# yenanjing/mmEgo

Hardware: AMD Instinct MI355X
Metric: train frames/sec (Upper+Lower U+L step, B=64/GPU, T=8, 128 pts) (higher is better)
Workload: dtype f32; 1 GPU; U+L step (Train_Upper + Train_Lower train_once bodies), B=64/GPU T=8 N=128, fp32, dropout live, two concurrent HIP-graph branches; global_batch=64, seq_len=8, points=128, parallelism=dp1

## Files before the change

### include/mmego_hip.h

```cpp
#ifndef MMEGO_HIP_H
#define MMEGO_HIP_H
#ifdef __cplusplus
extern "C" {
#endif

int mmego_gemm(void* stream, const float* A, long sam, long sak, const float* B, long sbk, long sbn, float* C,
               long scm, long scn, const float* bias, int M, int N, int K, int nbatch, long sAb, long sBb, long sCb,
               int relu, int accumulate, float* splitk_ws, int nsplit, long sBiasb, const float* cmul, float* asum);
typedef struct MmegoGemmDesc {
  const float* A; long sam, sak;
  const float* B; long sbk, sbn;
  float* C; long scm, scn;
  const float* bias;
  int M, N, K, nbatch;
  long sAb, sBb, sCb;
  int relu, accumulate;
  float* splitk_ws; int nsplit;
  long sBiasb;
  const float* cmul; float* asum;
} MmegoGemmDesc;
int mmego_gemm_group(void* stream, int n, const MmegoGemmDesc* descs);

int mmego_colstats_nblk(long rows);
int mmego_bn_train_stats(void* stream, const float* X, long ldx, long rows, int C, const float* gamma,
// ... 2 lines not shown
int mmego_bn_finalize(void* stream, const float* partial, int nblk, int C, const float* gamma, const float* beta,
                      float* running_mean, float* running_var, float momentum, float eps, float* mean, float* invstd, float* a,
                      float* b);
int mmego_bn_train_stats_pair(void* stream, long rows, int C, float* partial_ws,
                              const float* X1, long ldx1, const float* gamma1, const float* beta1, float* running_mean1,
                              float* running_var1, float momentum1, float eps1, float* mean1, float* invstd1, float* a1, float* b1,
                              const float* X2, long ldx2, const float* gamma2, const float* beta2, float* running_mean2,
                              float* running_var2, float momentum2, float eps2, float* mean2, float* invstd2, float* a2, float* b2);
int mmego_bn_eval_affine(void* stream, int C, const float* gamma, const float* beta, const float* running_mean,
                         const float* running_var, float eps, float* mean, float* invstd, float* a, float* b);
int mmego_bn_fold_linear(void* stream, const float* W, const float* b, int N, int K, const float* gamma, const float* beta,
                         const float* running_mean, const float* running_var, float eps, float* Wf, float* bf);
int mmego_mlp3_eval(void* stream, const float* X, long ldx, long rows, int Cin, const float* W1, const float* b1, int C1,
                    const float* W2, const float* b2, int C2, const float* W3, const float* b3, int C3, float* Y, long ldy,
                    const float* const* bn, float eps, int pre);
int mmego_mlp3_eval_bf16(void* stream, const float* X, long ldx, long rows, int Cin, const float* W1, const float* b1, int C1,
                         const float* W2, const float* b2, int C2, const float* W3, const float* b3, int C3, float* Y, long ldy,
                         const float* const* bn, float eps, int pre);
int mmego_affine_act(void* stream, const float* X1, long ld1, const float* m1, const float* a1, const float* b1,
                     const float* X2, long ld2, const float* m2, const float* a2, const float* b2, float* Y, long ldy,
                     long rows, int C, int relu);
int mmego_copy2d(void* stream, const float* X, long ldx, float* Y, long ldy, long rows, int C, int accumulate);
int mmego_gather_rows(void* stream, const float* X, long nsrc, long W, const long long* idx, long nout, float* Y);
int mmego_pack_frames(void* stream, const float* pts, const long long* frame_off, const long long* frame_idx, long nout,
                      int pc_no, int max_n, float keep_p, unsigned long long seed, float* out);
int mmego_pack_frames_noise(void* stream, const float* pts, const long long* frame_off, const long long* frame_idx, long nout,
                            int pc_no, int max_n, float keep_p, unsigned long long seed, float sigma_xyz, float sigma_v, float* out);
int mmego_pose_jitter(void* stream, const float* R, const float* t, long n, double sigma_deg, double sigma_t,
                      const long long* seed_word, const long long* ids, float* R_out, float* t_out);
int mmego_imu_jitter(void* stream, const float* imu, long n_rows, int T, int S,
                     double noise_rot_deg, double noise_acc, double noise_gyro,
                     double bias_rot_deg, double bias_acc, double bias_gyro,
                     const long long* seed_word, const long long* row_ids, const long long* win_ids,
                     float* out);
int mmego_blend_windows(void* stream, const float* src, long nrows, int C, const long long* cov_off, const int* cov_row,
                        const float* cov_w, long F, float* dst, long ldd, float* spread);
int mmego_colsum_phase(void* stream, const float* X, long ldx, long rows, int C, int period, float* out, long ldo);
int mmego_blend_bones(void* stream, const float* src, long nrows, int J, const long long* cov_off, const int* cov_row,
                      const float* cov_w, long F, const int* bones, const float* bone_len, int NB, float* dst, long ldd,
                      float* spread, int* fallback);
int mmego_bone_length_dev(void* stream, const float* X, long ldx, long n, int J, const int* bones, const float* bone_len, int NB,
                          float* out, long ldo);
int mmego_blend_rot(void* stream, const float* src, long nrows, int J, const float* q, int NQ, const float* Rh,
                    const long long* cov_off, const int* cov_row, const float* cov_w, long F, const int* bones, const int* rot_idx,
                    const float* body, int NB, float* dst, long ldd, float* quat, float* spread, float* rot_spread, int* fallback);
int mmego_smooth_frames(void* stream, const float* src, long lds, long F, int C, const int* seg, const float* w, int H, int D,
                        float* dst, long ldd, float* moved);
int mmego_smooth_bones(void* stream, const float* src, long lds, long F, int J, const int* seg, const float* w, int H, int D,
                       const int* bones, const float* bone_len, int NB, float* dst, long ldd, float* moved, int* fallback);
int mmego_floor_stats(void* stream, const float* lo, long ldl, const float* tgt, long ldt, const float* ground, const float* contact,
                      const int* seg, long rows, double H, float* out);
int mmego_floor_clamp(void* stream, const float* src, long lds, const float* ground, const int* seg, long rows, double margin, float* dst,
                      long ldd, float* lifted, int* fallback);
int mmego_bn_backward(void* stream, const float* dY, long lddy, const float* Ymask, long ldm, const float* X, long ldx,
                      const float* mean, const float* invstd, const float* a, long rows, int C, float* partial_ws,
                      float* c12_ws, float* dgamma, float* dbeta, float* dX, long lddx);
int mmego_bn_backward_pair(void* stream, const float* dY, long lddy, const float* Ymask, long ldm, long rows, int C,
                           float* partial_ws, float* c12_ws,
                           const float* X1, long ldx1, const float* mean1, const float* invstd1, const float* a1,
                           float* dgamma1, float* dbeta1, float* dX1, long lddx1,
                           const float* X2, long ldx2, const float* mean2, const float* invstd2, const float* a2,
                           float* dgamma2, float* dbeta2, float* dX2, long lddx2);
int mmego_colsum(void* stream, const float* X, long ldx, long rows, int C, float* partial_ws, float* out, float* out2,
                 int accumulate, const float* scale);
int mmego_colsum_pair(void* stream, const float* X, long ldx, long rows, int C, float* outA, float* outA2, float* outB,
                      float* outB2, int accumulate);
int mmego_relu_mask(void* stream, float* G, long ldg, const float* H, long ldh, long rows, int C);
int mmego_fill(void* stream, float* X, long n, float v);

int mmego_lstm_step(void* stream, int ndir, int Bn, int H, int first, const float* hprev0, const float* hprev1,
                    long hps, const float* whh0, const float* whh1, const float* bhh0, const float* bhh1,
                    const float* xproj0, const float* xproj1, long xs, float* hout0, float* hout1, long hos, float* c0,
                    float* c1, float* gst0, float* gst1, float* cst0, float* cst1);
int mmego_lstm64_forward(void* stream, int B, int T, const float* xproj0, const float* xproj1, long xs,
                         const float* whh0, const float* whh1, const float* bhh0, const float* bhh1, const float* h0_0,
                         const float* h0_1, const float* c0_0, const float* c0_1, float* out, long os, float* hn0,
                         float* hn1, float* cn0, float* cn1,
                         float* gates0, float* gates1, float* cst0, float* cst1, float* hprev0, float* hprev1,
                         float* drop_y, float* drop_mask, float drop_p, const unsigned long long* seed_ctr, int salt);
int mmego_lstm64_backward(void* stream, int B, int T, const float* dout, long dos, const float* gates0,
                          const float* gates1, const float* cst0, const float* cst1, const float* c0_0,
                          const float* c0_1, const float* whh0, const float* whh1, float* dgates0, float* dgates1,
                          long dgs);

typedef struct MmegoLstm64Fwd {
  const float* xproj[2]; long xs;
  const float* whh[2]; const float* bhh[2]; const float* h0[2]; const float* c0[2];
  float* out; long os;
  float* hn[2]; float* cn[2];
  float* gates[2]; float* cst[2]; float* hprev[2];
  int B, T;
  float* drop_y; float* drop_mask; float drop_p; const unsigned long long* seed_ctr; unsigned salt;
} MmegoLstm64Fwd;
typedef struct MmegoLstm64Bwd {
  const float* dout; long dos;
  const float* gates[2]; const float* cst[2]; const float* c0[2]; const float* whh[2];
  float* dgates[2]; long dgs;
  int B, T;
} MmegoLstm64Bwd;
int mmego_lstm64_forward_multi(void* stream, int n, const MmegoLstm64Fwd* descs);
int mmego_lstm64_backward_multi(void* stream, int n, const MmegoLstm64Bwd* descs);

int mmego_cvt_bf16(void* stream, const float* X, long ldx, long rows, long cols, unsigned short* Y, long ldy);
int mmego_cvt_bf16_tm(void* stream, const float* X, long ldx, int Bn, int T, long cols, unsigned short* Y, int Bp);
int mmego_gemm_bf16(void* stream, const unsigned short* A, long lda, const unsigned short* W, long ldw, float* C,
                    long ldc, unsigned short* Cb, long ldcb, float* Cf, const float* bias, int M, int N, int K, int relu);
int mmego_lstm_step_bf16(void* stream, int ndir, int Bn, int H, int first, const unsigned short* hprev0,
                         const unsigned short* hprev1, const unsigned short* whh0, const unsigned short* whh1,
                         const float* xpf, long mt0_0, long mt0_1, float* hout0, float* hout1,
                         long hos, unsigned short* houtb0, unsigned short* houtb1, long hbs,
                         unsigned short* hfrag0, unsigned short* hfrag1, float* c0, float* c1);

int mmego_lstm_step_bf16_fused(void* stream, int ndir, int Bn, int H, int first, int nseg,
                               const unsigned short* a0_0, const unsigned short* a0_1, const unsigned short* w0_0,
                               const unsigned short* w0_1, int K0, const unsigned short* a1_0,
                               const unsigned short* a1_1, const unsigned short* w1_0, const unsigned short* w1_1,
                               int K1, const unsigned short* hprev0, const unsigned short* hprev1,
                               const unsigned short* whh0, const unsigned short* whh1, const float* bias,
                               float* hout0, float* hout1, long hos, unsigned short* hfrag0, unsigned short* hfrag1,
                               float* c0, float* c1);
int mmego_attn_pool_frag_bf16_ok(int H);
int mmego_attn_pool_frag_bf16(void* stream, const unsigned short* hf, int T, int Bp, int Bn, int H, const float* w, const float* b,
                              float* vec, float* attn);
int mmego_cvt_bf16_frag_tm(void* stream, const float* X, long ldx, int Bn, int T, int C, unsigned short* Y, int Bp);
int mmego_fc_relu_bf16_frag_tm(void* stream, const float* X, long ldx, const float* W, const float* bias, int Bn, int T, int Cin,
                               int H, unsigned short* Y, int Bp, int relu);

int mmego_lstm_cell_backward(void* stream, int ndir, int Bn, int H, const float* dout0, const float* dout1, long dos,
                             const float* dhrec0, const float* dhrec1, const float* gst0, const float* gst1,
                             const float* cst0, const float* cst1, const float* cprev0, const float* cprev1, float* dc0,
                             float* dc1, float* dgates0, float* dgates1, long dgs);
int mmego_imu_loss(void* stream, const float* R, const float* t, const float* R_gt, const float* head_gt, long F,
                   float scale, float* loss, float* dR, float* dt);
int mmego_lstm_bwd_step(void* stream, int Bn, int H, const float* dg0, const float* dg1, long dgs, const float* wT0,
                        const float* wT1, const float* dout0, const float* dout1, long dos, const float* gst0,
                        const float* gst1, const float* cst0, const float* cst1, const float* cprev0, const float* cprev1,
                        float* dc0, float* dc1, float* dgo0, float* dgo1);
int mmego_imu_head_backward(void* stream, const float* y, const float* dR, const float* dt, long F, float* dy);

int mmego_transform2h(void* stream, float* pts, long F, int P, int C, const float* R, const float* t, const float* src,
                      long src_ld, float* keep, float* feats, long ldf, int nfeat);
int mmego_rotate_points(void* stream, const float* in, float* out, long F, int P, const float* R, const float* t,
                        int transpose, int add_t);
int mmego_transform2h_backward(void* stream, const float* pts, long ldp, long F, int P, const float* R, const float* t,
                               const float* g, long ldg, const float* g2, long ldg2, int accumulate, float* dR, float* dt);
int mmego_lower_inputs_backward(void* stream, const float* pts, long ldp, long F, int N, const long long* idx, int P, const float* R,
                                const float* t, const float* g, long ldg, const float* g2, long ldg2, const float* joints, int V,
                                const float* gj, long ldgj, const float* gj2, long ldgj2, int accumulate, float* dR, float* dt,
                                float* djoints);
int mmego_head_fk_forward(void* stream, int which, const float* y, const float* body, int B, long F, float* q,
                          float* joints, const float* Rw, const float* tw, float* world, long long* counters, int ncount,
                          unsigned long long* seed_ctr);
int mmego_head_fk_backward(void* stream, int which, const float* y, const float* body, int B, long F, const float* dj,
                           float* dy, const float* Rw);
int mmego_head_fk_backward_pose(void* stream, int which, const float* y, const float* body, int B, long F, const float* dj,
                                float* dy, const float* Rw, const float* joints_h, float* dRw, float* dtw);
int mmego_head_fk_backward_extra(void* stream, int which, const float* y, const float* body, int B, long F, const float* dj,
                                 float* dy, const float* Rw, const float* joints_h, float* dRw, float* dtw, const float* dR_add,
                                 const float* dt_add);
int mmego_head_fk_loss(void* stream, int which, const float* y, const float* body, int B, long F, float* q, float* joints_h,
                       const float* Rw, const float* tw, float* world, long long* counters, int ncount,
                       unsigned long long* seed_ctr, const float* target, const int* map, int ntgt, double scale, float* loss,
                       float* dy, double* scratch);
int mmego_head_fk_loss_pose(void* stream, int which, const float* y, const float* body, int B, long F, float* q, float* joints_h,
                            const float* Rw, const float* tw, float* world, long long* counters, int ncount,
                            unsigned long long* seed_ctr, const float* target, const int* map, int ntgt, double scale, float* loss,
// ... 257 lines not shown
```

### mmego_amd/csrc/lstm.hip

```cpp
#include "common.h"
#include "lstm_cell.h"
#include <stddef.h>
#include <string.h>

struct Lstm64P {
  const float* xproj[2]; long xs;
  const float* whh[2];
  const float* bhh[2];
  const float* h0[2]; const float* c0[2];
  float* out; long os;
  float* hn[2]; float* cn[2];
  float* gates[2]; float* cst[2]; float* hprev[2];
  int B, T;
  float* drop_y; float* drop_mask; float drop_p; const unsigned long long* seed_ctr; unsigned salt;
};
#define L64_SAME_FIELD(P, D, f) && offsetof(P, f) == offsetof(D, f) && sizeof(P::f) == sizeof(D::f)
#define L64_SAME_LAYOUT(P, D, FIELDS) static_assert(sizeof(P) == sizeof(D) FIELDS(L64_SAME_FIELD, P, D), #D " is " #P)
#define L64_FWD_FIELDS(X, P, D)                                                                                                        \
  X(P, D, xproj) X(P, D, xs) X(P, D, whh) X(P, D, bhh) X(P, D, h0) X(P, D, c0) X(P, D, out) X(P, D, os) X(P, D, hn) X(P, D, cn)       \
  X(P, D, gates) X(P, D, cst) X(P, D, hprev) X(P, D, B) X(P, D, T) X(P, D, drop_y) X(P, D, drop_mask) X(P, D, drop_p) X(P, D, seed_ctr) \
  X(P, D, salt)
L64_SAME_LAYOUT(Lstm64P, MmegoLstm64Fwd, L64_FWD_FIELDS);
template <class P, class D>
static inline P l64_param(const D& d) { P p; memcpy(&p, &d, sizeof p); return p; }


#define L64_LDS_BARRIER() asm volatile("s_waitcnt lgkmcnt(0)\n\ts_barrier" ::: "memory")

#define WLD 272

typedef const float __attribute__((address_space(1)))* l64_gcptr;
typedef float __attribute__((address_space(1)))* l64_gptr;
typedef f32x4 __attribute__((address_space(1)))* l64_gptr4;
typedef const f32x4 __attribute__((address_space(1)))* l64_gcptr4;

template <bool FULL, bool STASH, bool DROP>
__device__ __forceinline__ void lstm64_fwd_body(const Lstm64P& p) {
  extern __shared__ __attribute__((aligned(16))) float smem[];
  float* hs = smem;
  const int tid = threadIdx.x, lane = tid & 63, wave = tid >> 6;
  const int d = blockIdx.y, r0 = blockIdx.x * 16;
  const int B = p.B, T = p.T;
  const float* W = p.whh[d];
  const int fr = lane & 15, fq = lane >> 4;
  const int j = wave * 16 + fr;
  float creg[4], hreg[4], bh[4];
#pragma unroll
  for (int g = 0; g < 4; ++g) bh[g] = p.bhh[d] ? p.bhh[d][g * 64 + j] : 0.f;
#pragma unroll
  for (int reg = 0; reg < 4; ++reg) {
    int row = r0 + fq * 4 + reg;
    bool ok = row < B;
    creg[reg] = (ok && p.c0[d]) ? p.c0[d][row * 64 + j] : 0.f;
    hreg[reg] = (ok && p.h0[d]) ? p.h0[d][row * 64 + j] : 0.f;
    hs[j * 16 + fq * 4 + reg] = hreg[reg];
  }
  __syncthreads();
  float wreg[16][4];
#pragma unroll
  for (int g = 0; g < 4; ++g) {
    const float* wrow = W + (g * 64 + j) * 64 + 16 * fq;
#pragma unroll
    for (int q = 0; q < 4; ++q) {
      const f32x4 v = *reinterpret_cast<const f32x4*>(wrow + 4 * q);
      wreg[4 * q + 0][g] = v.x; wreg[4 * q + 1][g] = v.y; wreg[4 * q + 2][g] = v.z; wreg[4 * q + 3][g] = v.w;
    }
  }

  float xp[4][4], xpn[4][4];
  constexpr bool stash = STASH, keep_h = STASH, drop = DROP;
  const unsigned dkey = drop ? dropout_key(p.seed_ctr[0], p.salt) : 0u;
  const float keep_scale = drop ? 1.0f / (1.0f - p.drop_p) : 1.0f;
  const int t_first = d == 0 ? 0 : T - 1;
  const long dir = d == 0 ? 1 : -1;
  l64_gcptr xq[4];
  l64_gptr oq[4], hq[4], gq[4], cq[4];
  bool live[4];
#pragma unroll
  for (int reg = 0; reg < 4; ++reg) {
    const int row = r0 + fq * 4 + reg;
    live[reg] = FULL || row < B;
    const long rt = (long)(live[reg] ? row : 0) * T + t_first;
    xq[reg] = (l64_gcptr)(p.xproj[d] + rt * p.xs + j);
    oq[reg] = (l64_gptr)(p.out + rt * p.os + d * 64 + j);
    hq[reg] = keep_h ? (l64_gptr)(p.hprev[d] + rt * 64 + j) : (l64_gptr)nullptr;
    const long tr = (long)t_first * B + (live[reg] ? row : 0);
    gq[reg] = stash ? (l64_gptr)(p.gates[d] + tr * 256 + 4 * j) : (l64_gptr)nullptr;
    cq[reg] = stash ? (l64_gptr)(p.cst[d] + tr * 64 + j) : (l64_gptr)nullptr;
  }
  const long xstep = dir * p.xs, ostep = dir * p.os, hstep = dir * 64, gstep = dir * (long)B * 256,
             cstep = dir * (long)B * 64;
#define L64_LOAD_XP(DST)                                                                            \
  do {                                                                                              \
    _Pragma("unroll") for (int reg = 0; reg < 4; ++reg) {                                           \
      _Pragma("unroll") for (int g = 0; g < 4; ++g) DST[g][reg] = (FULL || live[reg]) ? xq[reg][g * 64] : 0.f; \
      xq[reg] += xstep;                                                                             \
    }                                                                                               \
  } while (0)
  L64_LOAD_XP(xp);
  for (int s = 0; s < T; ++s) {
    if (s + 1 >= T) {
#pragma unroll
      for (int reg = 0; reg < 4; ++reg) xq[reg] -= xstep;
    }
    L64_LOAD_XP(xpn);
    if (keep_h) {
#pragma unroll
      for (int reg = 0; reg < 4; ++reg) {
        if (FULL || live[reg]) *hq[reg] = hreg[reg];
        hq[reg] += hstep;
      }
    }
    f32x4 acc[4];
#pragma unroll
    for (int g = 0; g < 4; ++g) acc[g] = (f32x4){0.f, 0.f, 0.f, 0.f};
    float hk[16];
#pragma unroll
    for (int k4 = 0; k4 < 16; ++k4) hk[k4] = hs[(16 * fq + k4) * 16 + fr];
    __builtin_amdgcn_sched_barrier(0);
#pragma unroll
    for (int k4 = 0; k4 < 16; ++k4) {
#pragma unroll
      for (int g = 0; g < 4; ++g) acc[g] = __builtin_amdgcn_mfma_f32_16x16x4f32(hk[k4], wreg[k4][g], acc[g], 0, 0, 0);
    }
    L64_LDS_BARRIER();
#pragma unroll
    for (int reg = 0; reg < 4; ++reg) {
      const LstmCell u = lstm_cell_fwd(acc[0][reg] + (xp[0][reg] + bh[0]), acc[1][reg] + (xp[1][reg] + bh[1]),
                                       acc[2][reg] + (xp[2][reg] + bh[2]), acc[3][reg] + (xp[3][reg] + bh[3]), creg[reg]);
      const float cn = u.c, hn = u.h;
      creg[reg] = cn;
      hreg[reg] = hn;
      hs[j * 16 + fq * 4 + reg] = hn;
      if (FULL || live[reg]) {
        *oq[reg] = hn;
        if (drop) {
          const long off = oq[reg] - (l64_gptr)p.out;
          const float mk = dropout_keep(dkey, (unsigned)off, p.drop_p) ? keep_scale : 0.f;
          p.drop_mask[off] = mk;
          p.drop_y[off] = hn * mk;
        }
        if (stash) {
          *(l64_gptr4)gq[reg] = (f32x4){u.i, u.f, u.g, u.o};
          *cq[reg] = cn;
        }
      }
      oq[reg] += ostep;
      if (stash) { gq[reg] += gstep; cq[reg] += cstep; }
    }
    __builtin_amdgcn_sched_barrier(0);
#pragma unroll
    for (int g = 0; g < 4; ++g)
#pragma unroll
      for (int reg = 0; reg < 4; ++reg) xp[g][reg] = xpn[g][reg];
    L64_LDS_BARRIER();
  }
#undef L64_LOAD_XP
#pragma unroll
  for (int reg = 0; reg < 4; ++reg) {
    int row = r0 + fq * 4 + reg;
    if (row < B) {
      if (p.hn[d]) p.hn[d][row * 64 + j] = hreg[reg];
      if (p.cn[d]) p.cn[d][row * 64 + j] = creg[reg];
    }
  }
}

template <bool FULL, bool STASH, bool DROP>
__global__ __launch_bounds__(256) void lstm64_fwd_kernel(Lstm64P p) { lstm64_fwd_body<FULL, STASH, DROP>(p); }

#define L64_MAX_MULTI 4
struct Lstm64Multi { Lstm64P p[L64_MAX_MULTI]; };
template <bool FULL, bool STASH, bool DROP>
__global__ __launch_bounds__(256) void lstm64_fwd_multi_kernel(Lstm64Multi m) { lstm64_fwd_body<FULL, STASH, DROP>(m.p[blockIdx.z]); }

extern "C" int mmego_lstm64_forward(void* stream, int B, int T, const float* xproj0, const float* xproj1, long xs,
                                    const float* whh0, const float* whh1, const float* bhh0, const float* bhh1,
                                    const float* h0_0, const float* h0_1, const float* c0_0, const float* c0_1, float* out,
                                    long os, float* hn0, float* hn1,
                                    float* cn0, float* cn1, float* gates0, float* gates1, float* cst0, float* cst1,
                                    float* hprev0, float* hprev1, float* drop_y, float* drop_mask, float drop_p,
                                    const unsigned long long* seed_ctr, int salt) {
  MMEGO_REQUIRE((drop_mask == nullptr) == (drop_y == nullptr));
  MMEGO_REQUIRE(!drop_mask || (seed_ctr && drop_p > 0.f && drop_p < 1.f && (long)B * T * os < (1L << 32)));
  MMEGO_REQUIRE(B > 0 && T > 0 && xproj0 && xproj1 && whh0 && whh1 && out);
  MMEGO_REQUIRE((((uintptr_t)whh0 | (uintptr_t)whh1) & 15) == 0);
  MMEGO_REQUIRE((gates0 == nullptr) == (cst0 == nullptr) && (gates1 == nullptr) == (cst1 == nullptr));
  MMEGO_REQUIRE((((uintptr_t)gates0 | (uintptr_t)gates1) & 15) == 0);
  Lstm64P p;
  p.xproj[0] = xproj0; p.xproj[1] = xproj1; p.xs = xs;
  p.whh[0] = whh0; p.whh[1] = whh1;
  p.bhh[0] = bhh0; p.bhh[1] = bhh1;
  p.h0[0] = h0_0; p.h0[1] = h0_1; p.c0[0] = c0_0; p.c0[1] = c0_1;
  p.out = out; p.os = os;
  p.hn[0] = hn0; p.hn[1] = hn1; p.cn[0] = cn0; p.cn[1] = cn1;
  p.gates[0] = gates0; p.gates[1] = gates1; p.cst[0] = cst0; p.cst[1] = cst1;
  p.hprev[0] = hprev0; p.hprev[1] = hprev1;
  p.B = B; p.T = T;
  p.drop_y = drop_y; p.drop_mask = drop_mask; p.drop_p = drop_p; p.seed_ctr = seed_ctr; p.salt = (unsigned)salt;
  size_t lds = (size_t)(64 * 16) * sizeof(float);
  const bool full = B % 16 == 0, st_ = gates0 != nullptr, dr = drop_mask != nullptr;
  MMEGO_REQUIRE((hprev0 != nullptr) == st_ && (hprev1 != nullptr) == st_ && (gates1 != nullptr) == st_);
#define L64_FWD_LAUNCH(F_, S_, D_)                                                                                    \
  do {                                                                                                                \
    if (int e = mmego_allow_lds<lstm64_fwd_kernel<F_, S_, D_>>(lds)) return e;                                        \
    hipLaunchKernelGGL((lstm64_fwd_kernel<F_, S_, D_>), dim3(cdiv(B, 16), 2), dim3(256), lds, (hipStream_t)stream, p); \
  } while (0)
  if (full) {
    if (st_ && dr) L64_FWD_LAUNCH(true, true, true);
    else if (st_) L64_FWD_LAUNCH(true, true, false);
    else if (dr) L64_FWD_LAUNCH(true, false, true);
    else L64_FWD_LAUNCH(true, false, false);
  } else {
    if (st_ && dr) L64_FWD_LAUNCH(false, true, true);
    else if (st_) L64_FWD_LAUNCH(false, true, false);
    else if (dr) L64_FWD_LAUNCH(false, false, true);
    else L64_FWD_LAUNCH(false, false, false);
  }
#undef L64_FWD_LAUNCH
  MMEGO_LAUNCH_CHECK();
  return MMEGO_OK;
}

struct Lstm64BwdP {
  const float* dout; long dos;
  const float* gates[2]; const float* cst[2]; const float* c0[2];
  const float* whh[2];
  float* dgates[2]; long dgs;
  int B, T;
};
#define L64_BWD_FIELDS(X, P, D) \
  X(P, D, dout) X(P, D, dos) X(P, D, gates) X(P, D, cst) X(P, D, c0) X(P, D, whh) X(P, D, dgates) X(P, D, dgs) X(P, D, B) X(P, D, T)
L64_SAME_LAYOUT(Lstm64BwdP, MmegoLstm64Bwd, L64_BWD_FIELDS);

template <bool FULL>
__device__ __forceinline__ void lstm64_bwd_body(const Lstm64BwdP& p) {
  extern __shared__ __attribute__((aligned(16))) float smem[];
  float* dgs = smem;
  const int tid = threadIdx.x, lane = tid & 63, wave = tid >> 6;
  const int d = blockIdx.y, r0 = blockIdx.x * 16;
  const int B = p.B, T = p.T;
  const int fr = lane & 15, fq = lane >> 4;
  const int j = wave * 16 + fr;
  float wreg[64];
  {
    const float* W = p.whh[d] + fq * 64 + wave * 16 + fr;
#pragma unroll
    for (int i = 0; i < 64; ++i) wreg[i] = W[i * 256];
  }
  float dcreg[4] = {0.f, 0.f, 0.f, 0.f};
  f32x4 dhrec = {0.f, 0.f, 0.f, 0.f};

  float gin[4][6], gnx[4][6];
  float ccur[4];
  const l64_gcptr g_gates = (l64_gcptr)p.gates[d], g_dout = (l64_gcptr)p.dout, g_cst = (l64_gcptr)p.cst[d];
  const bool has_c0 = p.c0[d] != nullptr;
  const l64_gcptr g_c0 = has_c0 ? (l64_gcptr)p.c0[d] : g_cst;
#define L64_LOAD_BWD(DST, step)                                                                                \
  do {                                                                                                         \
    const int tq_ = d == 0 ? (step) : T - 1 - (step);                                                          \
    const int tp_ = d == 0 ? tq_ - 1 : tq_ + 1;                                                                \
    _Pragma("unroll") for (int reg = 0; reg < 4; ++reg) {                                                      \
      const int row_ = r0 + fq * 4 + reg;                                                                      \
      if (FULL || row_ < B) {                                                                                  \
        const f32x4 gv_ = *(l64_gcptr4)(g_gates + ((long)tq_ * B + row_) * 256 + 4 * j);                       \
        DST[reg][0] = g_dout[((long)row_ * T + tq_) * p.dos + d * 64 + j];                                     \
        DST[reg][1] = gv_.x; DST[reg][2] = gv_.y; DST[reg][3] = gv_.z; DST[reg][4] = gv_.w;                    \
        const l64_gcptr cp_ = ((step) > 0) ? g_cst + ((long)tp_ * B + row_) * 64 + j : g_c0 + (long)row_ * 64 + j; \
        const float cv_ = *cp_;                                                                                \
        DST[reg][5] = ((step) > 0 || has_c0) ? cv_ : 0.f;                                                      \
      } else {                                                                                                 \
        _Pragma("unroll") for (int q = 0; q < 6; ++q) DST[reg][q] = 0.f;                                       \
      }                                                                                                        \
    }                                                                                                          \
  } while (0)
  L64_LOAD_BWD(gin, T - 1);
  {
    const int tl = d == 0 ? T - 1 : 0;
#pragma unroll
    for (int reg = 0; reg < 4; ++reg) {
      int row = r0 + fq * 4 + reg;
      ccur[reg] = (FULL || row < B) ? g_cst[((long)tl * B + row) * 64 + j] : 0.f;
    }
  }
  for (int s = T - 1; s >= 0; --s) {
    const int tt = d == 0 ? s : T - 1 - s;
    const int sn = s > 0 ? s - 1 : 0;
    L64_LOAD_BWD(gnx, sn);
    float dg4[4][4];
#pragma unroll
    for (int reg = 0; reg < 4; ++reg) {
      int row = r0 + fq * 4 + reg;
      if (FULL || row < B) {
        float dh = gin[reg][0] + dhrec[reg];
        float gi = gin[reg][1], gf = gin[reg][2], gg = gin[reg][3], go = gin[reg][4];
        const LstmCellGrad o = lstm_cell_bwd(gi, gf, gg, go, fast_tanh(ccur[reg]), gin[reg][5], dcreg[reg], dh);
        dg4[0][reg] = o.di;
        dg4[1][reg] = o.df;
        dg4[2][reg] = o.dg;
        dg4[3][reg] = o.dout;
        dcreg[reg] = o.dcprev;
        l64_gptr dst = (l64_gptr)p.dgates[d] + ((long)row * T + tt) * p.dgs + j;
#pragma unroll
        for (int g = 0; g < 4; ++g) dst[g * 64] = dg4[g][reg];
      } else {
#pragma unroll
        for (int g = 0; g < 4; ++g) dg4[g][reg] = 0.f;
      }
#pragma unroll
      for (int g = 0; g < 4; ++g) dgs[(g * 64 + j) * 16 + fq * 4 + reg] = dg4[g][reg];
      ccur[reg] = gin[reg][5];
    }
    L64_LDS_BARRIER();
    f32x4 a0 = {0.f, 0.f, 0.f, 0.f}, a1 = {0.f, 0.f, 0.f, 0.f}, a2 = {0.f, 0.f, 0.f, 0.f}, a3 = {0.f, 0.f, 0.f, 0.f};
#pragma unroll
    for (int nb = 0; nb < 64; nb += 16) {
      float dk[16];
#pragma unroll
      for (int u = 0; u < 16; ++u) dk[u] = dgs[((nb + u) * 4 + fq) * 16 + fr];
      __builtin_amdgcn_sched_barrier(0);
#pragma unroll
      for (int u = 0; u < 16; u += 4) {
        a0 = __builtin_amdgcn_mfma_f32_16x16x4f32(dk[u], wreg[nb + u], a0, 0, 0, 0);
        a1 = __builtin_amdgcn_mfma_f32_16x16x4f32(dk[u + 1], wreg[nb + u + 1], a1, 0, 0, 0);
        a2 = __builtin_amdgcn_mfma_f32_16x16x4f32(dk[u + 2], wreg[nb + u + 2], a2, 0, 0, 0);
        a3 = __builtin_amdgcn_mfma_f32_16x16x4f32(dk[u + 3], wreg[nb + u + 3], a3, 0, 0, 0);
      }
    }
    dhrec = (a0 + a1) + (a2 + a3);
    __builtin_amdgcn_sched_barrier(0);
#pragma unroll
    for (int reg = 0; reg < 4; ++reg)
#pragma unroll
      for (int q = 0; q < 6; ++q) gin[reg][q] = gnx[reg][q];
    L64_LDS_BARRIER();
  }
#undef L64_LOAD_BWD
}

template <bool FULL>
__global__ __launch_bounds__(256) void lstm64_bwd_kernel(Lstm64BwdP p) { lstm64_bwd_body<FULL>(p); }
struct Lstm64BwdMulti { Lstm64BwdP p[L64_MAX_MULTI]; };
template <bool FULL>
__global__ __launch_bounds__(256) void lstm64_bwd_multi_kernel(Lstm64BwdMulti m) { lstm64_bwd_body<FULL>(m.p[blockIdx.z]); }

extern "C" int mmego_lstm64_backward(void* stream, int B, int T, const float* dout, long dos, const float* gates0,
                                     const float* gates1, const float* cst0, const float* cst1, const float* c0_0,
                                     const float* c0_1, const float* whh0, const float* whh1, float* dgates0,
                                     float* dgates1, long dgs) {
  MMEGO_REQUIRE(B > 0 && T > 0 && dout && gates0 && gates1 && cst0 && cst1 && whh0 && whh1 && dgates0 && dgates1);
  MMEGO_REQUIRE((((uintptr_t)whh0 | (uintptr_t)whh1) & 15) == 0);
  MMEGO_REQUIRE((((uintptr_t)gates0 | (uintptr_t)gates1) & 15) == 0);
  Lstm64BwdP p;
  p.dout = dout; p.dos = dos;
  p.gates[0] = gates0; p.gates[1] = gates1; p.cst[0] = cst0; p.cst[1] = cst1;
  p.c0[0] = c0_0; p.c0[1] = c0_1;
  p.whh[0] = whh0; p.whh[1] = whh1;
  p.dgates[0] = dgates0; p.dgates[1] = dgates1; p.dgs = dgs;
  p.B = B; p.T = T;
  const size_t lds = (size_t)(256 * 16) * sizeof(float);
  if (B % 16 == 0) hipLaunchKernelGGL(lstm64_bwd_kernel<true>, dim3(cdiv(B, 16), 2), dim3(256), lds, (hipStream_t)stream, p);
  else hipLaunchKernelGGL(lstm64_bwd_kernel<false>, dim3(cdiv(B, 16), 2), dim3(256), lds, (hipStream_t)stream, p);
  MMEGO_LAUNCH_CHECK();
  return MMEGO_OK;
}

extern "C" int mmego_lstm64_forward_multi(void* stream, int n, const MmegoLstm64Fwd* h) {
  MMEGO_REQUIRE(h && n >= 1 && n <= L64_MAX_MULTI);
  Lstm64Multi m;
  const int B = h[0].B, T = h[0].T;
  const bool st_ = h[0].gates[0] != nullptr, dr = h[0].drop_mask != nullptr;
  for (int i = 0; i < n; ++i) {
    const MmegoLstm64Fwd& p = h[i];
    MMEGO_REQUIRE(p.B == B && p.T == T && B > 0 && T > 0 && p.xproj[0] && p.xproj[1] && p.whh[0] && p.whh[1] && p.out);
    MMEGO_REQUIRE((((uintptr_t)p.whh[0] | (uintptr_t)p.whh[1]) & 15) == 0);
    MMEGO_REQUIRE((((uintptr_t)p.gates[0] | (uintptr_t)p.gates[1]) & 15) == 0);
    MMEGO_REQUIRE((p.drop_mask == nullptr) == (p.drop_y == nullptr) && (p.drop_mask != nullptr) == dr);
    MMEGO_REQUIRE(!p.drop_mask || (p.seed_ctr && p.drop_p > 0.f && p.drop_p < 1.f && (long)B * T * p.os < (1L << 32)));
    MMEGO_REQUIRE((p.gates[0] != nullptr) == st_ && (p.gates[1] != nullptr) == st_ && (p.cst[0] != nullptr) == st_ && (p.cst[1] != nullptr) == st_ &&
                  (p.hprev[0] != nullptr) == st_ && (p.hprev[1] != nullptr) == st_);
    m.p[i] = l64_param<Lstm64P>(p);
  }
  for (int i = n; i < L64_MAX_MULTI; ++i) m.p[i] = m.p[0];
  const size_t lds = (size_t)(64 * 16) * sizeof(float);
  const bool full = B % 16 == 0;
#define L64_FWDM_LAUNCH(F_, S_, D_) hipLaunchKernelGGL((lstm64_fwd_multi_kernel<F_, S_, D_>), dim3(cdiv(B, 16), 2, n), dim3(256), lds, (hipStream_t)stream, m)
  if (full) {
    if (st_ && dr) L64_FWDM_LAUNCH(true, true, true);
    else if (st_) L64_FWDM_LAUNCH(true, true, false);
    else if (dr) L64_FWDM_LAUNCH(true, false, true);
    else L64_FWDM_LAUNCH(true, false, false);
  } else {
    if (st_ && dr) L64_FWDM_LAUNCH(false, true, true);
    else if (st_) L64_FWDM_LAUNCH(false, true, false);
    else if (dr) L64_FWDM_LAUNCH(false, false, true);
    else L64_FWDM_LAUNCH(false, false, false);
  }
#undef L64_FWDM_LAUNCH
  MMEGO_LAUNCH_CHECK();
  return MMEGO_OK;
}

extern "C" int mmego_lstm64_backward_multi(void* stream, int n, const MmegoLstm64Bwd* h) {
  MMEGO_REQUIRE(h && n >= 1 && n <= L64_MAX_MULTI);
  Lstm64BwdMulti m;
  const int B = h[0].B, T = h[0].T;
  for (int i = 0; i < n; ++i) {
    const MmegoLstm64Bwd& p = h[i];
    MMEGO_REQUIRE(p.B == B && p.T == T && B > 0 && T > 0 && p.dout && p.gates[0] && p.gates[1] && p.cst[0] && p.cst[1] && p.whh[0] && p.whh[1] &&
                  p.dgates[0] && p.dgates[1]);
    MMEGO_REQUIRE((((uintptr_t)p.whh[0] | (uintptr_t)p.whh[1]) & 15) == 0);
    MMEGO_REQUIRE((((uintptr_t)p.gates[0] | (uintptr_t)p.gates[1]) & 15) == 0);
    m.p[i] = l64_param<Lstm64BwdP>(p);
  }
  for (int i = n; i < L64_MAX_MULTI; ++i) m.p[i] = m.p[0];
  const size_t lds = (size_t)(256 * 16) * sizeof(float);
  if (B % 16 == 0) hipLaunchKernelGGL(lstm64_bwd_multi_kernel<true>, dim3(cdiv(B, 16), 2, n), dim3(256), lds, (hipStream_t)stream, m);
  else hipLaunchKernelGGL(lstm64_bwd_multi_kernel<false>, dim3(cdiv(B, 16), 2, n), dim3(256), lds, (hipStream_t)stream, m);
  MMEGO_LAUNCH_CHECK();
  return MMEGO_OK;
}
```

Before: 105,300 frames/s.

## Add 4-row LSTM64 workgroup variant using 4x4 MFMA to spread batch across CUs

```diff
diff --git a/include/mmego_hip.h b/include/mmego_hip.h
--- a/include/mmego_hip.h
+++ b/include/mmego_hip.h
@@ -108,6 +108,7 @@
                           const float* gates1, const float* cst0, const float* cst1, const float* c0_0,
                           const float* c0_1, const float* whh0, const float* whh1, float* dgates0, float* dgates1,
                           long dgs);
+int mmego_lstm64_rows(int B);
 
 typedef struct MmegoLstm64Fwd {
   const float* xproj[2]; long xs;
diff --git a/mmego_amd/csrc/lstm.hip b/mmego_amd/csrc/lstm.hip
--- a/mmego_amd/csrc/lstm.hip
+++ b/mmego_amd/csrc/lstm.hip
@@ -1,6 +1,7 @@
 #include "common.h"
 #include "lstm_cell.h"
 #include <stddef.h>
+#include <stdlib.h>
 #include <string.h>
 
 struct Lstm64P {
@@ -34,51 +35,139 @@
 typedef f32x4 __attribute__((address_space(1)))* l64_gptr4;
 typedef const f32x4 __attribute__((address_space(1)))* l64_gcptr4;
 
-template <bool FULL, bool STASH, bool DROP>
+template <int ROWS>
+struct L64Map {
+  static_assert(ROWS == 16 || ROWS == 4, "rows of a workgroup");
+  static constexpr int RPL = ROWS / 4;
+  static __device__ __forceinline__ int unit(int wave, int lane) { return wave * 16 + (ROWS == 16 ? (lane & 15) : (lane >> 2)); }
+  static __device__ __forceinline__ int row0(int lane) { return ROWS == 16 ? (lane >> 4) * 4 : (lane & 3); }
+};
+
+template <int ABID>
+__device__ __forceinline__ f32x4 l64_mfma4(float a, float b, f32x4 c) { return __builtin_amdgcn_mfma_f32_4x4x1f32(a, b, c, 4, ABID, 0); }
+#define L64_X16(X) X(0) X(1) X(2) X(3) X(4) X(5) X(6) X(7) X(8) X(9) X(10) X(11) X(12) X(13) X(14) X(15)
+
+__device__ __forceinline__ float l64_quad_perm_b1(float v) { return __int_as_float(__builtin_amdgcn_update_dpp(0, __float_as_int(v), 0xB1, 0xF, 0xF, true)); }
+__device__ __forceinline__ float l64_quad_perm_4e(float v) { return __int_as_float(__builtin_amdgcn_update_dpp(0, __float_as_int(v), 0x4E, 0xF, 0xF, true)); }
+__device__ __forceinline__ void l64_quad_transpose(float (&a)[4], int lane) {
+  const bool o1 = lane & 1, o2 = lane & 2;
+#pragma unroll
+  for (int r = 0; r < 4; r += 2) {
+    const float x = a[r], y = a[r + 1], got = l64_quad_perm_b1(o1 ? x : y);
+    a[r] = o1 ? got : x;
+    a[r + 1] = o1 ? y : got;
+  }
+#pragma unroll
+  for (int q = 0; q < 2; ++q) {
+    const float x = a[q], y = a[q + 2], got = l64_quad_perm_4e(o2 ? x : y);
+    a[q] = o2 ? got : x;
+    a[q + 2] = o2 ? y : got;
+  }
+}
+
+template <int ROWS>
+struct L64FwdProd;
+template <>
+struct L64FwdProd<16> {
+  float wreg[16][4];
+  __device__ __forceinline__ void load(const float* W, int wave, int lane) {
+    const int fq = lane >> 4, j = wave * 16 + (lane & 15);
+#pragma unroll
+    for (int g = 0; g < 4; ++g) {
+      const float* wrow = W + (g * 64 + j) * 64 + 16 * fq;
+#pragma unroll
+      for (int q = 0; q < 4; ++q) {
+        const f32x4 v = *reinterpret_cast<const f32x4*>(wrow + 4 * q);
+        wreg[4 * q + 0][g] = v.x; wreg[4 * q + 1][g] = v.y; wreg[4 * q + 2][g] = v.z; wreg[4 * q + 3][g] = v.w;
+      }
+    }
+  }
+  __device__ __forceinline__ void run(const float* hs, int lane, float (&pre)[4][4]) const {
+    const int fr = lane & 15, fq = lane >> 4;
+    f32x4 acc[4];
+#pragma unroll
+    for (int g = 0; g < 4; ++g) acc[g] = (f32x4){0.f, 0.f, 0.f, 0.f};
+    float hk[16];
+#pragma unroll
+    for (int k4 = 0; k4 < 16; ++k4) hk[k4] = hs[(16 * fq + k4) * 16 + fr];
+    __builtin_amdgcn_sched_barrier(0);
+#pragma unroll
+    for (int k4 = 0; k4 < 16; ++k4) {
+#pragma unroll
+      for (int g = 0; g < 4; ++g) acc[g] = __builtin_amdgcn_mfma_f32_16x16x4f32(hk[k4], wreg[k4][g], acc[g], 0, 0, 0);
+    }
+#pragma unroll
+    for (int g = 0; g < 4; ++g)
+#pragma unroll
+      for (int reg = 0; reg < 4; ++reg) pre[g][reg] = acc[g][reg];
+  }
+};
+template <>
+struct L64FwdProd<4> {
+  float wreg[64];
+  __device__ __forceinline__ void load(const float* W, int wave, int lane) {
+    const float* wrow = W + ((lane & 3) * 64 + wave * 16 + (lane >> 2)) * 64;
+#pragma unroll
+    for (int q = 0; q < 16; ++q) {
+      const f32x4 v = *reinterpret_cast<const f32x4*>(wrow + 4 * q);
+      wreg[4 * q + 0] = v.x; wreg[4 * q + 1] = v.y; wreg[4 * q + 2] = v.z; wreg[4 * q + 3] = v.w;
+    }
+  }
+  __device__ __forceinline__ void run(const float* hs, int lane, float (&pre)[4][1]) const {
+    f32x4 s = {0.f, 0.f, 0.f, 0.f};
+    float hk[4];
+#pragma unroll
+    for (int v = 0; v < 4; ++v) hk[v] = hs[64 * v + lane];
+    __builtin_amdgcn_sched_barrier(0);
+#define L64_FWD_K(A_)                                                                                                       \
+  s = l64_mfma4<A_>(hk[0], wreg[A_], s); s = l64_mfma4<A_>(hk[1], wreg[16 + A_], s); s = l64_mfma4<A_>(hk[2], wreg[32 + A_], s); \
+  s = l64_mfma4<A_>(hk[3], wreg[48 + A_], s);
+    L64_X16(L64_FWD_K)
+#undef L64_FWD_K
+    float a[4] = {s.x, s.y, s.z, s.w};
+    l64_quad_transpose(a, lane);
+#pragma unroll
+    for (int g = 0; g < 4; ++g) pre[g][0] = a[g];
+  }
+};
+
+template <bool FULL, bool STASH, bool DROP, int ROWS>
 __device__ __forceinline__ void lstm64_fwd_body(const Lstm64P& p) {
   extern __shared__ __attribute__((aligned(16))) float smem[];
+  using Map = L64Map<ROWS>;
+  constexpr int R = Map::RPL;
   float* hs = smem;
   const int tid = threadIdx.x, lane = tid & 63, wave = tid >> 6;
-  const int d = blockIdx.y, r0 = blockIdx.x * 16;
+  const int d = blockIdx.y, r0 = blockIdx.x * ROWS;
   const int B = p.B, T = p.T;
-  const float* W = p.whh[d];
-  const int fr = lane & 15, fq = lane >> 4;
-  const int j = wave * 16 + fr;
-  float creg[4], hreg[4], bh[4];
+  const int j = Map::unit(wave, lane), rl = Map::row0(lane);
+  float creg[R], hreg[R], bh[4];
 #pragma unroll
   for (int g = 0; g < 4; ++g) bh[g] = p.bhh[d] ? p.bhh[d][g * 64 + j] : 0.f;
 #pragma unroll
-  for (int reg = 0; reg < 4; ++reg) {
-    int row = r0 + fq * 4 + reg;
+  for (int reg = 0; reg < R; ++reg) {
+    int row = r0 + rl + reg;
     bool ok = row < B;
     creg[reg] = (ok && p.c0[d]) ? p.c0[d][row * 64 + j] : 0.f;
     hreg[reg] = (ok && p.h0[d]) ? p.h0[d][row * 64 + j] : 0.f;
-    hs[j * 16 + fq * 4 + reg] = hreg[reg];
+    hs[j * ROWS + rl + reg] = hreg[reg];
   }
   __syncthreads();
-  float wreg[16][4];
-#pragma unroll
-  for (int g = 0; g < 4; ++g) {
-    const float* wrow = W + (g * 64 + j) * 64 + 16 * fq;
-#pragma unroll
-    for (int q = 0; q < 4; ++q) {
-      const f32x4 v = *reinterpret_cast<const f32x4*>(wrow + 4 * q);
-      wreg[4 * q + 0][g] = v.x; wreg[4 * q + 1][g] = v.y; wreg[4 * q + 2][g] = v.z; wreg[4 * q + 3][g] = v.w;
-    }
-  }
-
-  float xp[4][4], xpn[4][4];
+  L64FwdProd<ROWS> prod;
+  prod.load(p.whh[d], wave, lane);
+
+  float xp[4][R], xpn[4][R];
   constexpr bool stash = STASH, keep_h = STASH, drop = DROP;
   const unsigned dkey = drop ? dropout_key(p.seed_ctr[0], p.salt) : 0u;
   const float keep_scale = drop ? 1.0f / (1.0f - p.drop_p) : 1.0f;
   const int t_first = d == 0 ? 0 : T - 1;
   const long dir = d == 0 ? 1 : -1;
-  l64_gcptr xq[4];
-  l64_gptr oq[4], hq[4], gq[4], cq[4];
-  bool live[4];
-#pragma unroll
-  for (int reg = 0; reg < 4; ++reg) {
-    const int row = r0 + fq * 4 + reg;
+  l64_gcptr xq[R];
+  l64_gptr oq[R], hq[R], gq[R], cq[R];
+  bool live[R];
+#pragma unroll
+  for (int reg = 0; reg < R; ++reg) {
+    const int row = r0 + rl + reg;
     live[reg] = FULL || row < B;
     const long rt = (long)(live[reg] ? row : 0) * T + t_first;
     xq[reg] = (l64_gcptr)(p.xproj[d] + rt * p.xs + j);
@@ -92,7 +181,7 @@
              cstep = dir * (long)B * 64;
 #define L64_LOAD_XP(DST)                                                                            \
   do {                                                                                              \
-    _Pragma("unroll") for (int reg = 0; reg < 4; ++reg) {                                           \
+    _Pragma("unroll") for (int reg = 0; reg < R; ++reg) {                                           \
       _Pragma("unroll") for (int g = 0; g < 4; ++g) DST[g][reg] = (FULL || live[reg]) ? xq[reg][g * 64] : 0.f; \
       xq[reg] += xstep;                                                                             \
     }                                                                                               \
@@ -101,37 +190,27 @@
   for (int s = 0; s < T; ++s) {
     if (s + 1 >= T) {
 #pragma unroll
-      for (int reg = 0; reg < 4; ++reg) xq[reg] -= xstep;
+      for (int reg = 0; reg < R; ++reg) xq[reg] -= xstep;
     }
     L64_LOAD_XP(xpn);
     if (keep_h) {
 #pragma unroll
-      for (int reg = 0; reg < 4; ++reg) {
+      for (int reg = 0; reg < R; ++reg) {
         if (FULL || live[reg]) *hq[reg] = hreg[reg];
         hq[reg] += hstep;
       }
     }
-    f32x4 acc[4];
-#pragma unroll
-    for (int g = 0; g < 4; ++g) acc[g] = (f32x4){0.f, 0.f, 0.f, 0.f};
-    float hk[16];
-#pragma unroll
-    for (int k4 = 0; k4 < 16; ++k4) hk[k4] = hs[(16 * fq + k4) * 16 + fr];
-    __builtin_amdgcn_sched_barrier(0);
-#pragma unroll
-    for (int k4 = 0; k4 < 16; ++k4) {
-#pragma unroll
-      for (int g = 0; g < 4; ++g) acc[g] = __builtin_amdgcn_mfma_f32_16x16x4f32(hk[k4], wreg[k4][g], acc[g], 0, 0, 0);
-    }
+    float acc[4][R];
+    prod.run(hs, lane, acc);
     L64_LDS_BARRIER();
 #pragma unroll
-    for (int reg = 0; reg < 4; ++reg) {
+    for (int reg = 0; reg < R; ++reg) {
       const LstmCell u = lstm_cell_fwd(acc[0][reg] + (xp[0][reg] + bh[0]), acc[1][reg] + (xp[1][reg] + bh[1]),
                                        acc[2][reg] + (xp[2][reg] + bh[2]), acc[3][reg] + (xp[3][reg] + bh[3]), creg[reg]);
       const float cn = u.c, hn = u.h;
       creg[reg] = cn;
       hreg[reg] = hn;
-      hs[j * 16 + fq * 4 + reg] = hn;
+      hs[j * ROWS + rl + reg] = hn;
       if (FULL || live[reg]) {
         *oq[reg] = hn;
         if (drop) {
@@ -152,13 +231,13 @@
 #pragma unroll
     for (int g = 0; g < 4; ++g)
 #pragma unroll
-      for (int reg = 0; reg < 4; ++reg) xp[g][reg] = xpn[g][reg];
+      for (int reg = 0; reg < R; ++reg) xp[g][reg] = xpn[g][reg];
     L64_LDS_BARRIER();
   }
 #undef L64_LOAD_XP
 #pragma unroll
-  for (int reg = 0; reg < 4; ++reg) {
-    int row = r0 + fq * 4 + reg;
+  for (int reg = 0; reg < R; ++reg) {
+    int row = r0 + rl + reg;
     if (row < B) {
       if (p.hn[d]) p.hn[d][row * 64 + j] = hreg[reg];
       if (p.cn[d]) p.cn[d][row * 64 + j] = creg[reg];
@@ -166,13 +245,21 @@
   }
 }
 
-template <bool FULL, bool STASH, bool DROP>
-__global__ __launch_bounds__(256) void lstm64_fwd_kernel(Lstm64P p) { lstm64_fwd_body<FULL, STASH, DROP>(p); }
+template <bool FULL, bool STASH, bool DROP, int ROWS>
+__global__ __launch_bounds__(256) void lstm64_fwd_kernel(Lstm64P p) { lstm64_fwd_body<FULL, STASH, DROP, ROWS>(p); }
 
 #define L64_MAX_MULTI 4
 struct Lstm64Multi { Lstm64P p[L64_MAX_MULTI]; };
-template <bool FULL, bool STASH, bool DROP>
-__global__ __launch_bounds__(256) void lstm64_fwd_multi_kernel(Lstm64Multi m) { lstm64_fwd_body<FULL, STASH, DROP>(m.p[blockIdx.z]); }
+template <bool FULL, bool STASH, bool DROP, int ROWS>
+__global__ __launch_bounds__(256) void lstm64_fwd_multi_kernel(Lstm64Multi m) { lstm64_fwd_body<FULL, STASH, DROP, ROWS>(m.p[blockIdx.z]); }
+
+static int l64_rows(int B) {
+  const char* env = getenv("MMEGO_LSTM64_ROWS");
+  const int forced = env ? atoi(env) : 0;
+  if (forced == 4 || forced == 16) return forced;
+  return 2 * cdiv(B, 16) * 2 <= mmego_cu_count() ? 4 : 16;
+}
+extern "C" int mmego_lstm64_rows(int B) { return B > 0 ? l64_rows(B) : MMEGO_EBADARG; }
 
 extern "C" int mmego_lstm64_forward(void* stream, int B, int T, const float* xproj0, const float* xproj1, long xs,
                                     const float* whh0, const float* whh1, const float* bhh0, const float* bhh1,
@@ -198,14 +285,16 @@
   p.hprev[0] = hprev0; p.hprev[1] = hprev1;
   p.B = B; p.T = T;
   p.drop_y = drop_y; p.drop_mask = drop_mask; p.drop_p = drop_p; p.seed_ctr = seed_ctr; p.salt = (unsigned)salt;
-  size_t lds = (size_t)(64 * 16) * sizeof(float);
-  const bool full = B % 16 == 0, st_ = gates0 != nullptr, dr = drop_mask != nullptr;
+  const int rows = l64_rows(B);
+  size_t lds = (size_t)(64 * rows) * sizeof(float);
+  const bool full = B % rows == 0, st_ = gates0 != nullptr, dr = drop_mask != nullptr;
   MMEGO_REQUIRE((hprev0 != nullptr) == st_ && (hprev1 != nullptr) == st_ && (gates1 != nullptr) == st_);
-#define L64_FWD_LAUNCH(F_, S_, D_)                                                                                    \
-  do {                                                                                                                \
-    if (int e = mmego_allow_lds<lstm64_fwd_kernel<F_, S_, D_>>(lds)) return e;                                        \
-    hipLaunchKernelGGL((lstm64_fwd_kernel<F_, S_, D_>), dim3(cdiv(B, 16), 2), dim3(256), lds, (hipStream_t)stream, p); \
+#define L64_FWD_LAUNCH_R(F_, S_, D_, R_)                                                                                     \
+  do {                                                                                                                       \
+    if (int e = mmego_allow_lds<lstm64_fwd_kernel<F_, S_, D_, R_>>(lds)) return e;                                           \
+    hipLaunchKernelGGL((lstm64_fwd_kernel<F_, S_, D_, R_>), dim3(cdiv(B, R_), 2), dim3(256), lds, (hipStream_t)stream, p);   \
   } while (0)
+#define L64_FWD_LAUNCH(F_, S_, D_) do { if (rows == 4) L64_FWD_LAUNCH_R(F_, S_, D_, 4); else L64_FWD_LAUNCH_R(F_, S_, D_, 16); } while (0)
   if (full) {
     if (st_ && dr) L64_FWD_LAUNCH(true, true, true);
     else if (st_) L64_FWD_LAUNCH(true, true, false);
@@ -218,6 +307,7 @@
     else L64_FWD_LAUNCH(false, false, false);
   }
 #undef L64_FWD_LAUNCH
+#undef L64_FWD_LAUNCH_R
   MMEGO_LAUNCH_CHECK();
   return MMEGO_OK;
 }
@@ -233,26 +323,102 @@
   X(P, D, dout) X(P, D, dos) X(P, D, gates) X(P, D, cst) X(P, D, c0) X(P, D, whh) X(P, D, dgates) X(P, D, dgs) X(P, D, B) X(P, D, T)
 L64_SAME_LAYOUT(Lstm64BwdP, MmegoLstm64Bwd, L64_BWD_FIELDS);
 
-template <bool FULL>
+template <int ROWS>
+struct L64BwdProd;
+template <>
+struct L64BwdProd<16> {
+  static constexpr int LDS_FLOATS = 256 * 16;
+  static __device__ __forceinline__ int at(int n, int row) { return n * 16 + row; }
+  float wreg[64];
+  f32x4 dh4;
+  __device__ __forceinline__ void load(const float* Whh, int wave, int lane) {
+    const float* W = Whh + (lane >> 4) * 64 + wave * 16 + (lane & 15);
+#pragma unroll
+    for (int i = 0; i < 64; ++i) wreg[i] = W[i * 256];
+  }
+  __device__ __forceinline__ void run(float* dgs, int wave, int lane) {
+    const int fr = lane & 15, fq = lane >> 4;
+    f32x4 a0 = {0.f, 0.f, 0.f, 0.f}, a1 = {0.f, 0.f, 0.f, 0.f}, a2 = {0.f, 0.f, 0.f, 0.f}, a3 = {0.f, 0.f, 0.f, 0.f};
+#pragma unroll
+    for (int nb = 0; nb < 64; nb += 16) {
+      float dk[16];
+#pragma unroll
+      for (int u = 0; u < 16; ++u) dk[u] = dgs[((nb + u) * 4 + fq) * 16 + fr];
+      __builtin_amdgcn_sched_barrier(0);
+#pragma unroll
+      for (int u = 0; u < 16; u += 4) {
+        a0 = __builtin_amdgcn_mfma_f32_16x16x4f32(dk[u], wreg[nb + u], a0, 0, 0, 0);
+        a1 = __builtin_amdgcn_mfma_f32_16x16x4f32(dk[u + 1], wreg[nb + u + 1], a1, 0, 0, 0);
+        a2 = __builtin_amdgcn_mfma_f32_16x16x4f32(dk[u + 2], wreg[nb + u + 2], a2, 0, 0, 0);
+        a3 = __builtin_amdgcn_mfma_f32_16x16x4f32(dk[u + 3], wreg[nb + u + 3], a3, 0, 0, 0);
+      }
+    }
+    dh4 = (a0 + a1) + (a2 + a3);
+  }
+  __device__ __forceinline__ void take(const float* dgs, int wave, int lane, float (&dh)[4]) const {
+#pragma unroll
+    for (int reg = 0; reg < 4; ++reg) dh[reg] = dh4[reg];
+  }
+};
+template <>
+struct L64BwdProd<4> {
+  static constexpr int WLDS = 272, PART = 4 * WLDS, PLD = 72, LDS_FLOATS = PART + 4 * 4 * PLD;
+  static __device__ __forceinline__ int at(int n, int row) { return ((n & 15) >> 2) * WLDS + (4 * (n >> 4) + (n & 3)) * 4 + row; }
+  float wreg[64];
+  __device__ __forceinline__ void load(const float* Whh, int wave, int lane) {
+    const float* W = Whh + (long)(4 * wave) * 64 + lane;
+#pragma unroll
+    for (int i = 0; i < 64; ++i) wreg[i] = W[(16 * (i >> 2) + (i & 3)) * 64];
+  }
+  __device__ __forceinline__ void run(float* dgs, int wave, int lane) {
+    f32x4 s = {0.f, 0.f, 0.f, 0.f};
+    float dk[4];
+#pragma unroll
+    for (int v = 0; v < 4; ++v) dk[v] = dgs[WLDS * wave + 64 * v + lane];
+    __builtin_amdgcn_sched_barrier(0);
+#define L64_BWD_K(A_) s = l64_mfma4<A_>(dk[V_], wreg[16 * V_ + A_], s);
+#define V_ 0
+    L64_X16(L64_BWD_K)
+#undef V_
+#define V_ 1
+    L64_X16(L64_BWD_K)
+#undef V_
+#define V_ 2
+    L64_X16(L64_BWD_K)
+#undef V_
+#define V_ 3
+    L64_X16(L64_BWD_K)
+#undef V_
+#undef L64_BWD_K
+    float* part = dgs + PART + wave * (4 * PLD) + lane;
+#pragma unroll
+    for (int i = 0; i < 4; ++i) part[i * PLD] = s[i];
+  }
+  __device__ __forceinline__ void take(const float* dgs, int wave, int lane, float (&dh)[1]) const {
+    const float* part = dgs + PART + (lane & 3) * PLD + wave * 16 + (lane >> 2);
+    const float p0 = part[0], p1 = part[4 * PLD], p2 = part[8 * PLD], p3 = part[12 * PLD];
+    dh[0] = (p0 + p1) + (p2 + p3);
+  }
+};
+
+template <bool FULL, int ROWS>
 __device__ __forceinline__ void lstm64_bwd_body(const Lstm64BwdP& p) {
   extern __shared__ __attribute__((aligned(16))) float smem[];
+  using Map = L64Map<ROWS>;
+  constexpr int R = Map::RPL;
   float* dgs = smem;
   const int tid = threadIdx.x, lane = tid & 63, wave = tid >> 6;
-  const int d = blockIdx.y, r0 = blockIdx.x * 16;
+  const int d = blockIdx.y, r0 = blockIdx.x * ROWS;
   const int B = p.B, T = p.T;
-  const int fr = lane & 15, fq = lane >> 4;
-  const int j = wave * 16 + fr;
-  float wreg[64];
-  {
-    const float* W = p.whh[d] + fq * 64 + wave * 16 + fr;
-#pragma unroll
-    for (int i = 0; i < 64; ++i) wreg[i] = W[i * 256];
-  }
-  float dcreg[4] = {0.f, 0.f, 0.f, 0.f};
-  f32x4 dhrec = {0.f, 0.f, 0.f, 0.f};
-
-  float gin[4][6], gnx[4][6];
-  float ccur[4];
+  const int j = Map::unit(wave, lane), rl = Map::row0(lane);
+  L64BwdProd<ROWS> prod;
+  prod.load(p.whh[d], wave, lane);
+  float dcreg[R], dhrec[R];
+#pragma unroll
+  for (int reg = 0; reg < R; ++reg) dcreg[reg] = dhrec[reg] = 0.f;
+
+  float gin[R][6], gnx[R][6];
+  float ccur[R];
   const l64_gcptr g_gates = (l64_gcptr)p.gates[d], g_dout = (l64_gcptr)p.dout, g_cst = (l64_gcptr)p.cst[d];
   const bool has_c0 = p.c0[d] != nullptr;
   const l64_gcptr g_c0 = has_c0 ? (l64_gcptr)p.c0[d] : g_cst;
@@ -260,8 +426,8 @@
   do {                                                                                                         \
     const int tq_ = d == 0 ? (step) : T - 1 - (step);                                                          \
     const int tp_ = d == 0 ? tq_ - 1 : tq_ + 1;                                                                \
-    _Pragma("unroll") for (int reg = 0; reg < 4; ++reg) {                                                      \
-      const int row_ = r0 + fq * 4 + reg;                                                                      \
+    _Pragma("unroll") for (int reg = 0; reg < R; ++reg) {                                                      \
+      const int row_ = r0 + rl + reg;                                                                          \
       if (FULL || row_ < B) {                                                                                  \
         const f32x4 gv_ = *(l64_gcptr4)(g_gates + ((long)tq_ * B + row_) * 256 + 4 * j);                       \
         DST[reg][0] = g_dout[((long)row_ * T + tq_) * p.dos + d * 64 + j];                                     \
@@ -278,8 +444,8 @@
   {
     const int tl = d == 0 ? T - 1 : 0;
 #pragma unroll
-    for (int reg = 0; reg < 4; ++reg) {
-      int row = r0 + fq * 4 + reg;
+    for (int reg = 0; reg < R; ++reg) {
+      int row = r0 + rl + reg;
       ccur[reg] = (FULL || row < B) ? g_cst[((long)tl * B + row) * 64 + j] : 0.f;
     }
   }
@@ -287,10 +453,10 @@
     const int tt = d == 0 ? s : T - 1 - s;
     const int sn = s > 0 ? s - 1 : 0;
     L64_LOAD_BWD(gnx, sn);
-    float dg4[4][4];
-#pragma unroll
-    for (int reg = 0; reg < 4; ++reg) {
-      int row = r0 + fq * 4 + reg;
+    float dg4[4][R];
+#pragma unroll
+    for (int reg = 0; reg < R; ++reg) {
+      int row = r0 + rl + reg;
       if (FULL || row < B) {
         float dh = gin[reg][0] + dhrec[reg];
         float gi = gin[reg][1], gf = gin[reg][2], gg = gin[reg][3], go = gin[reg][4];
@@ -308,41 +474,27 @@
         for (int g = 0; g < 4; ++g) dg4[g][reg] = 0.f;
       }
 #pragma unroll
-      for (int g = 0; g < 4; ++g) dgs[(g * 64 + j) * 16 + fq * 4 + reg] = dg4[g][reg];
+      for (int g = 0; g < 4; ++g) dgs[L64BwdProd<ROWS>::at(g * 64 + j, rl + reg)] = dg4[g][reg];
       ccur[reg] = gin[reg][5];
     }
     L64_LDS_BARRIER();
-    f32x4 a0 = {0.f, 0.f, 0.f, 0.f}, a1 = {0.f, 0.f, 0.f, 0.f}, a2 = {0.f, 0.f, 0.f, 0.f}, a3 = {0.f, 0.f, 0.f, 0.f};
-#pragma unroll
-    for (int nb = 0; nb < 64; nb += 16) {
-      float dk[16];
-#pragma unroll
-      for (int u = 0; u < 16; ++u) dk[u] = dgs[((nb + u) * 4 + fq) * 16 + fr];
-      __builtin_amdgcn_sched_barrier(0);
-#pragma unroll
-      for (int u = 0; u < 16; u += 4) {
-        a0 = __builtin_amdgcn_mfma_f32_16x16x4f32(dk[u], wreg[nb + u], a0, 0, 0, 0);
-        a1 = __builtin_amdgcn_mfma_f32_16x16x4f32(dk[u + 1], wreg[nb + u + 1], a1, 0, 0, 0);
-        a2 = __builtin_amdgcn_mfma_f32_16x16x4f32(dk[u + 2], wreg[nb + u + 2], a2, 0, 0, 0);
-        a3 = __builtin_amdgcn_mfma_f32_16x16x4f32(dk[u + 3], wreg[nb + u + 3], a3, 0, 0, 0);
-      }
-    }
-    dhrec = (a0 + a1) + (a2 + a3);
+    prod.run(dgs, wave, lane);
     __builtin_amdgcn_sched_barrier(0);
 #pragma unroll
-    for (int reg = 0; reg < 4; ++reg)
+    for (int reg = 0; reg < R; ++reg)
 #pragma unroll
       for (int q = 0; q < 6; ++q) gin[reg][q] = gnx[reg][q];
     L64_LDS_BARRIER();
+    prod.take(dgs, wave, lane, dhrec);
   }
 #undef L64_LOAD_BWD
 }
 
-template <bool FULL>
-__global__ __launch_bounds__(256) void lstm64_bwd_kernel(Lstm64BwdP p) { lstm64_bwd_body<FULL>(p); }
+template <bool FULL, int ROWS>
+__global__ __launch_bounds__(256) void lstm64_bwd_kernel(Lstm64BwdP p) { lstm64_bwd_body<FULL, ROWS>(p); }
 struct Lstm64BwdMulti { Lstm64BwdP p[L64_MAX_MULTI]; };
-template <bool FULL>
-__global__ __launch_bounds__(256) void lstm64_bwd_multi_kernel(Lstm64BwdMulti m) { lstm64_bwd_body<FULL>(m.p[blockIdx.z]); }
+template <bool FULL, int ROWS>
+__global__ __launch_bounds__(256) void lstm64_bwd_multi_kernel(Lstm64BwdMulti m) { lstm64_bwd_body<FULL, ROWS>(m.p[blockIdx.z]); }
 
 extern "C" int mmego_lstm64_backward(void* stream, int B, int T, const float* dout, long dos, const float* gates0,
                                      const float* gates1, const float* cst0, const float* cst1, const float* c0_0,
@@ -358,9 +510,14 @@
   p.whh[0] = whh0; p.whh[1] = whh1;
   p.dgates[0] = dgates0; p.dgates[1] = dgates1; p.dgs = dgs;
   p.B = B; p.T = T;
-  const size_t lds = (size_t)(256 * 16) * sizeof(float);
-  if (B % 16 == 0) hipLaunchKernelGGL(lstm64_bwd_kernel<true>, dim3(cdiv(B, 16), 2), dim3(256), lds, (hipStream_t)stream, p);
-  else hipLaunchKernelGGL(lstm64_bwd_kernel<false>, dim3(cdiv(B, 16), 2), dim3(256), lds, (hipStream_t)stream, p);
+#define L64_BWD_LAUNCH(K_, R_, Z_, P_)                                                                                              \
+  do {                                                                                                                              \
+    const size_t lds = (size_t)L64BwdProd<R_>::LDS_FLOATS * sizeof(float);                                                          \
+    if (B % R_ == 0) hipLaunchKernelGGL((K_<true, R_>), dim3(cdiv(B, R_), 2, Z_), dim3(256), lds, (hipStream_t)stream, P_);         \
+    else hipLaunchKernelGGL((K_<false, R_>), dim3(cdiv(B, R_), 2, Z_), dim3(256), lds, (hipStream_t)stream, P_);                    \
+  } while (0)
+  if (l64_rows(B) == 4) L64_BWD_LAUNCH(lstm64_bwd_kernel, 4, 1, p);
+  else L64_BWD_LAUNCH(lstm64_bwd_kernel, 16, 1, p);
   MMEGO_LAUNCH_CHECK();
   return MMEGO_OK;
 }
@@ -382,9 +539,11 @@
     m.p[i] = l64_param<Lstm64P>(p);
   }
   for (int i = n; i < L64_MAX_MULTI; ++i) m.p[i] = m.p[0];
-  const size_t lds = (size_t)(64 * 16) * sizeof(float);
-  const bool full = B % 16 == 0;
-#define L64_FWDM_LAUNCH(F_, S_, D_) hipLaunchKernelGGL((lstm64_fwd_multi_kernel<F_, S_, D_>), dim3(cdiv(B, 16), 2, n), dim3(256), lds, (hipStream_t)stream, m)
+  const int rows = l64_rows(B);
+  const size_t lds = (size_t)(64 * rows) * sizeof(float);
+  const bool full = B % rows == 0;
+#define L64_FWDM_LAUNCH_R(F_, S_, D_, R_) hipLaunchKernelGGL((lstm64_fwd_multi_kernel<F_, S_, D_, R_>), dim3(cdiv(B, R_), 2, n), dim3(256), lds, (hipStream_t)stream, m)
+#define L64_FWDM_LAUNCH(F_, S_, D_) do { if (rows == 4) L64_FWDM_LAUNCH_R(F_, S_, D_, 4); else L64_FWDM_LAUNCH_R(F_, S_, D_, 16); } while (0)
   if (full) {
     if (st_ && dr) L64_FWDM_LAUNCH(true, true, true);
     else if (st_) L64_FWDM_LAUNCH(true, true, false);
@@ -397,6 +556,7 @@
     else L64_FWDM_LAUNCH(false, false, false);
   }
 #undef L64_FWDM_LAUNCH
+#undef L64_FWDM_LAUNCH_R
   MMEGO_LAUNCH_CHECK();
   return MMEGO_OK;
 }
@@ -414,9 +574,9 @@
     m.p[i] = l64_param<Lstm64BwdP>(p);
   }
   for (int i = n; i < L64_MAX_MULTI; ++i) m.p[i] = m.p[0];
-  const size_t lds = (size_t)(256 * 16) * sizeof(float);
-  if (B % 16 == 0) hipLaunchKernelGGL(lstm64_bwd_multi_kernel<true>, dim3(cdiv(B, 16), 2, n), dim3(256), lds, (hipStream_t)stream, m);
-  else hipLaunchKernelGGL(lstm64_bwd_multi_kernel<false>, dim3(cdiv(B, 16), 2, n), dim3(256), lds, (hipStream_t)stream, m);
+  if (l64_rows(B) == 4) L64_BWD_LAUNCH(lstm64_bwd_multi_kernel, 4, n, m);
+  else L64_BWD_LAUNCH(lstm64_bwd_multi_kernel, 16, n, m);
+#undef L64_BWD_LAUNCH
   MMEGO_LAUNCH_CHECK();
   return MMEGO_OK;
 }
```

Measured after the change: 107,400 frames/s, median of 6. +2.0%, better.
